# araffin/srl-zoo

Measured on AMD Instinct MI355X. Metric: images/sec (224x224x3) AE+VAE train step, higher is better.
Workload: dtype f32; 1 GPU; synthetic 224x224x3 obs, --losses autoencoder, custom_cnn, state-dim 200, bs=256 per GPU (512 frames fwd+bwd per step per GPU), Adam lr 0.005, normalised fp32 observations resident in HBM; global_batch=256, parallelism=dp1, rccl_ranks=1, devices=1

## Files before the change

srl-zoo_amd/csrc/bn_pool.hip:

```cpp
#include "common.h"

namespace {

constexpr int STAGE_ROWS = 128;

template <typename T>
__global__ __launch_bounds__(256) void reduce_rows_kernel(const T* __restrict__ rows, int nrows, double* __restrict__ out) {
  rows += (size_t)blockIdx.y * nrows * 128;
  out += (size_t)blockIdx.y * gridDim.x * 128;
  const int col = threadIdx.x & 127, half = threadIdx.x >> 7;
  double a0 = 0.0, a1 = 0.0, a2 = 0.0, a3 = 0.0;
  const int step = 2 * gridDim.x;
  int r = blockIdx.x * 2 + half;
  for (; r + 3 * step < nrows; r += 4 * step) {
    a0 += (double)rows[(size_t)r * 128 + col];
    a1 += (double)rows[(size_t)(r + step) * 128 + col];
    a2 += (double)rows[(size_t)(r + 2 * step) * 128 + col];
    a3 += (double)rows[(size_t)(r + 3 * step) * 128 + col];
  }
  for (; r < nrows; r += step) a0 += (double)rows[(size_t)r * 128 + col];
  __shared__ double sm[128];
  const double s = (a0 + a1) + (a2 + a3);
  if (half) sm[col] = s;
  __syncthreads();
  if (!half) out[(size_t)blockIdx.x * 128 + col] = s + sm[col];
}

static int stage_blocks(int nrows) {
  int g = (nrows + 7) / 8;
  if (g > STAGE_ROWS) g = STAGE_ROWS;
  return g < 1 ? 1 : g;
}

__global__ __launch_bounds__(1024) void bn_finalize_kernel(const double* __restrict__ partial, int n_partials, double count,
                                   const float* __restrict__ gamma, const float* __restrict__ beta, float eps,
                                   float momentum, int repeat, float* __restrict__ running_mean,
                                   float* __restrict__ running_var, float* __restrict__ bnp,
                                   float* __restrict__ batch_stat, int groups, long long* __restrict__ tick) {
  if (tick && blockIdx.x == 0 && threadIdx.x == 0) tick[0] += groups;
  gamma += blockIdx.x * 64; beta += blockIdx.x * 64;
  if (running_mean) running_mean += blockIdx.x * 64;
  if (running_var) running_var += blockIdx.x * 64;
  bnp += blockIdx.x * 256;
  partial += (size_t)blockIdx.x * groups * n_partials * 128;
  const int rec_stride = 256 * (int)gridDim.x;
  constexpr int NP = 16;
  const int c = threadIdx.x & 63, part = threadIdx.x >> 6;
  __shared__ double sm[2][NP][64];
  float rm = 0.f, rv = 0.f;
  const bool upd = running_mean && running_var;
  if (part == 0 && upd) { rm = running_mean[c]; rv = running_var[c]; }
  for (int g = 0; g < groups; ++g) {
    const double* pg = partial + (size_t)g * n_partials * 128;
    double s = 0.0, q = 0.0;
    for (int i = part; i < n_partials; i += NP) {
      s += pg[(size_t)i * 128 + c];
      q += pg[(size_t)i * 128 + 64 + c];
    }
    __syncthreads();
    sm[0][part][c] = s; sm[1][part][c] = q;
    __syncthreads();
    if (part == 0) {
      s = 0.0; q = 0.0;
#pragma unroll
      for (int k = 0; k < NP; ++k) { s += sm[0][k][c]; q += sm[1][k][c]; }
      const double mean = s / count;
      double var = q / count - mean * mean;
      if (var < 0.0) var = 0.0;
      const float invstd = (float)(1.0 / sqrt(var + (double)eps));
      const float ga = gamma[c], be = beta[c];
      const float scale = ga * invstd;
      float* rec = bnp + g * rec_stride;
      rec[c] = (float)mean; rec[64 + c] = invstd; rec[128 + c] = scale; rec[192 + c] = be - (float)mean * scale;
      const double unbiased = (count > 1.0) ? var * count / (count - 1.0) : var;
      if (batch_stat) { batch_stat[g * 128 + c] = (float)mean; batch_stat[g * 128 + 64 + c] = (float)unbiased; }
      for (int r = 0; r < repeat; ++r) {
        rm = (1.f - momentum) * rm + momentum * (float)mean;
        rv = (1.f - momentum) * rv + momentum * (float)unbiased;
      }
    }
  }
  if (part == 0 && upd) { running_mean[c] = rm; running_var[c] = rv; }
}

__global__ void bn_eval_params_kernel(const float* gamma, const float* beta, const float* rm, const float* rv, float eps,
                                      float* bnp) {
  const int c = threadIdx.x;
  const float invstd = 1.f / sqrtf(rv[c] + eps);
  const float scale = gamma[c] * invstd;
  bnp[c] = rm[c]; bnp[64 + c] = invstd; bnp[128 + c] = scale; bnp[192 + c] = beta[c] - rm[c] * scale;
}

__global__ void bn_replay_kernel(const float* batch_stat, float momentum, float* rm, float* rv) {
  const int c = threadIdx.x;
  rm[c] = (1.f - momentum) * rm[c] + momentum * batch_stat[c];
  rv[c] = (1.f - momentum) * rv[c] + momentum * batch_stat[64 + c];
}

__global__ __launch_bounds__(256) void bn_relu_pool_fwd_kernel(const float* __restrict__ y, const float* __restrict__ bnp,
                                                               float* __restrict__ pooled, uint8_t* __restrict__ argmax,
                                                               int N, int H, int W, int HP, int WP, int pad, int out_nchw,
                                                               int npg, int gx) {
  const int HB = (HP + 1) >> 1, WB = (WP + 1) >> 1;
  const int t = xcd_remap(blockIdx.x, gridDim.x);
  const int brow = t / gx, xb = t - brow * gx;
  const int c4 = threadIdx.x & 15;
  const int bx = (xb * blockDim.x + threadIdx.x) >> 4;
  if (bx >= WB) return;
  const int n = brow / HB, by = brow - n * HB;
  bnp += (n / npg) * 256;
  const f32x4 sc = *(const f32x4*)(bnp + 128 + c4 * 4);
  const f32x4 sh = *(const f32x4*)(bnp + 192 + c4 * 4);
  const int py0 = 2 * by, px0 = 2 * bx;
  const int iy0 = py0 * 2 - pad, ix0 = px0 * 2 - pad;
  f32x4 win[25];
  unsigned inside = 0;
#pragma unroll
  for (int r = 0; r < 5; ++r)
#pragma unroll
    for (int c = 0; c < 5; ++c) {
      const int iy = iy0 + r, ix = ix0 + c;
      const bool ok = iy >= 0 && iy < H && ix >= 0 && ix < W;
      win[r * 5 + c] = *(const f32x4*)(y + (ok ? ((size_t)(n * H + iy) * W + ix) * 64 : (size_t)0) + c4 * 4);
      inside |= (ok ? 1u : 0u) << (r * 5 + c);
    }
#pragma unroll
  for (int k = 0; k < 25; ++k) {
#pragma unroll
    for (int j = 0; j < 4; ++j) {
      float z = win[k][j] * sc[j] + sh[j];
      win[k][j] = z > 0.f ? z : 0.f;
    }
  }
#pragma unroll
  for (int dy = 0; dy < 2; ++dy)
#pragma unroll
    for (int dx = 0; dx < 2; ++dx) {
      const int py = py0 + dy, px = px0 + dx;
      if (py >= HP || px >= WP) continue;
      f32x4 best = {-1.f, -1.f, -1.f, -1.f};
      int bi[4] = {0, 0, 0, 0};
#pragma unroll
      for (int ky = 0; ky < 3; ++ky)
#pragma unroll
        for (int kx = 0; kx < 3; ++kx) {
          const int e = (2 * dy + ky) * 5 + 2 * dx + kx;
          const bool ok = (inside >> e) & 1u;
#pragma unroll
          for (int j = 0; j < 4; ++j)
            if (ok && win[e][j] > best[j]) { best[j] = win[e][j]; bi[j] = ky * 3 + kx; }
        }
      const long long pix = ((long long)n * HP + py) * WP + px;
      if (out_nchw) {
#pragma unroll
        for (int j = 0; j < 4; ++j) pooled[((size_t)(n * 64 + c4 * 4 + j) * HP + py) * WP + px] = best[j];
      } else {
        *(f32x4*)(pooled + (size_t)pix * 64 + c4 * 4) = best;
      }
      if (argmax) {
        const uint32_t packed = (uint32_t)bi[0] | ((uint32_t)bi[1] << 8) | ((uint32_t)bi[2] << 16) | ((uint32_t)bi[3] << 24);
        *(uint32_t*)(argmax + (size_t)pix * 64 + c4 * 4) = packed;
      }
    }
}

__device__ __forceinline__ void block_reduce_store(const double (&s1)[4], const double (&s2)[4], double* __restrict__ partial) {
  __shared__ double sm[16][128];
  const int c4 = threadIdx.x & 15, prow = threadIdx.x >> 4;
#pragma unroll
  for (int j = 0; j < 4; ++j) { sm[prow][c4 * 4 + j] = s1[j]; sm[prow][64 + c4 * 4 + j] = s2[j]; }
  __syncthreads();
  if (threadIdx.x < 128) {
    double s = 0.0;
#pragma unroll
    for (int r = 0; r < 16; ++r) s += sm[r][threadIdx.x];
    partial[((size_t)blockIdx.y * gridDim.x + blockIdx.x) * 128 + threadIdx.x] = s;
  }
}

__global__ __launch_bounds__(256) void bn_relu_pool_bwd_reduce(const float* __restrict__ y, const float* __restrict__ bnp,
                                                              const uint8_t* __restrict__ argmax,
                                                              const float* __restrict__ dpooled,
                                                              const float* __restrict__ pooled, double* __restrict__ partial,
                                                              int N, int H, int W, int HP, int WP, int pad, int dp_nchw) {
  bnp += blockIdx.y * 256;
  const int n0 = blockIdx.y * N;
  const int c4 = threadIdx.x & 15;
  const f32x4 mean = *(const f32x4*)(bnp + c4 * 4);
  const f32x4 invstd = *(const f32x4*)(bnp + 64 + c4 * 4);
  const f32x4 sc = *(const f32x4*)(bnp + 128 + c4 * 4);
  const f32x4 sh = *(const f32x4*)(bnp + 192 + c4 * 4);
  double s1[4] = {0.0, 0.0, 0.0, 0.0}, s2[4] = {0.0, 0.0, 0.0, 0.0};
  for (int lrow = blockIdx.x; lrow < N * HP; lrow += gridDim.x) {
    const int row = n0 * HP + lrow;
    const int n = row / HP, py = row - n * HP;
    for (int px = threadIdx.x >> 4; px < WP; px += 16) {
      const long long pix = (long long)row * WP + px;
      const uint32_t packed = *(const uint32_t*)(argmax + (size_t)pix * 64 + c4 * 4);
      f32x4 dp;
      if (dp_nchw) {
#pragma unroll
        for (int j = 0; j < 4; ++j) dp[j] = dpooled[((size_t)(n * 64 + c4 * 4 + j) * HP + py) * WP + px];
      } else {
        dp = *(const f32x4*)(dpooled + (size_t)pix * 64 + c4 * 4);
      }
      f32x4 pz = {0.f, 0.f, 0.f, 0.f};
      if (pooled) {
        if (dp_nchw) {
#pragma unroll
          for (int j = 0; j < 4; ++j) pz[j] = pooled[((size_t)(n * 64 + c4 * 4 + j) * HP + py) * WP + px];
        } else {
          pz = *(const f32x4*)(pooled + (size_t)pix * 64 + c4 * 4);
        }
      }
#pragma unroll
      for (int j = 0; j < 4; ++j) {
        float v, z;
        if (pooled && fabsf(sc[j]) > 1e-3f * fabsf(sh[j])) {
          z = pz[j];
          v = (z - sh[j]) / sc[j];
        } else {
          const int a = (packed >> (8 * j)) & 0xff;
          const int iy = py * 2 - pad + a / 3, ix = px * 2 - pad + a % 3;
          v = y[((size_t)(n * H + iy) * W + ix) * 64 + c4 * 4 + j];
          z = v * sc[j] + sh[j];
        }
        if (z > 0.f) {
          s1[j] += (double)dp[j];
          s2[j] += (double)(dp[j] * ((v - mean[j]) * invstd[j]));
        }
      }
    }
  }
  block_reduce_store(s1, s2, partial);
}

__global__ __launch_bounds__(1024) void bn_bwd_finalize(const double* __restrict__ partial, int nblocks, float* __restrict__ sums,
                                                       float* __restrict__ dgamma, float* __restrict__ dbeta, int groups) {
  const int c = threadIdx.x & 127, part = threadIdx.x >> 7;
  __shared__ double sm[8][128];
  double total = 0.0;
  for (int g = 0; g < groups; ++g) {
    const double* pg = partial + (size_t)g * nblocks * 128;
    double s = 0.0;
    for (int i = part; i < nblocks; i += 8) s += pg[(size_t)i * 128 + c];
    __syncthreads();
    sm[part][c] = s;
    __syncthreads();
    if (part == 0) {
      s = ((sm[0][c] + sm[1][c]) + (sm[2][c] + sm[3][c])) + ((sm[4][c] + sm[5][c]) + (sm[6][c] + sm[7][c]));
      sums[g * 128 + c] = (float)s;
      total = (g == 0) ? s : total + s;
    }
  }
  if (part == 0) {
    if (c < 64) { if (dbeta) dbeta[c] = (float)total; } else { if (dgamma) dgamma[c - 64] = (float)total; }
  }
}

__global__ __launch_bounds__(256) void bn_relu_pool_bwd_apply(const float* __restrict__ y, const float* __restrict__ bnp,
                                                             const uint8_t* __restrict__ argmax,
                                                             const float* __restrict__ dpooled, const float* __restrict__ sums,
                                                             float* __restrict__ dy, int N, int H, int W, int HP, int WP,
                                                             int pad, int dp_nchw, int training, float inv_count, int npg, int gx) {
  const int HB = (H + pad + 1) / 2, WB = (W + pad + 1) / 2;
  {
    const int t = xcd_remap(blockIdx.x, gridDim.x);
    const int brow = t / gx, xb = t - brow * gx;
    const int c4 = threadIdx.x & 15;
    const int bx = (xb * blockDim.x + threadIdx.x) >> 4;
    if (bx >= WB) return;
    const int n = brow / HB, by = brow - n * HB;
    bnp += (n / npg) * 256;
    sums += (n / npg) * 128;
    const f32x4 mean = *(const f32x4*)(bnp + c4 * 4);
    const f32x4 invstd = *(const f32x4*)(bnp + 64 + c4 * 4);
    const f32x4 sc = *(const f32x4*)(bnp + 128 + c4 * 4);
    const f32x4 sh = *(const f32x4*)(bnp + 192 + c4 * 4);
    f32x4 m1 = {0.f, 0.f, 0.f, 0.f}, m2 = m1;
    if (training) { m1 = *(const f32x4*)(sums + c4 * 4); m2 = *(const f32x4*)(sums + 64 + c4 * 4); }
    uint32_t am[2][2];
    f32x4 dp[2][2];
    unsigned wok = 0;
#pragma unroll
    for (int a = 0; a < 2; ++a)
#pragma unroll
      for (int b = 0; b < 2; ++b) {
        const int py = by - 1 + a, px = bx - 1 + b;
        const bool ok = py >= 0 && py < HP && px >= 0 && px < WP;
        const size_t pp = ok ? ((size_t)(n * HP + py) * WP + px) : (size_t)0;
        am[a][b] = *(const uint32_t*)(argmax + pp * 64 + c4 * 4);
        if (dp_nchw) {
#pragma unroll
          for (int j = 0; j < 4; ++j)
            dp[a][b][j] = dpooled[ok ? ((size_t)(n * 64 + c4 * 4 + j) * HP + py) * WP + px : (size_t)0];
        } else {
          dp[a][b] = *(const f32x4*)(dpooled + pp * 64 + c4 * 4);
        }
        wok |= (ok ? 1u : 0u) << (2 * a + b);
      }
    f32x4 yv[2][2];
    unsigned yok = 0;
#pragma unroll
    for (int ry = 0; ry < 2; ++ry)
#pragma unroll
      for (int rx = 0; rx < 2; ++rx) {
        const int iy = 2 * by - pad + ry, ix = 2 * bx - pad + rx;
        const bool ok = iy >= 0 && iy < H && ix >= 0 && ix < W;
        yv[ry][rx] = *(const f32x4*)(y + (ok ? ((size_t)(n * H + iy) * W + ix) * 64 : (size_t)0) + c4 * 4);
        yok |= (ok ? 1u : 0u) << (2 * ry + rx);
      }
#pragma unroll
    for (int a = 0; a < 2; ++a)
#pragma unroll
      for (int b = 0; b < 2; ++b) {
        asm volatile("" : "+v"(am[a][b]), "+v"(dp[a][b]), "+v"(yv[a][b]));
        if (!((wok >> (2 * a + b)) & 1u)) am[a][b] = 0xffffffffu;
      }
#pragma unroll
    for (int ry = 0; ry < 2; ++ry) {
      const int iy = 2 * by - pad + ry;
#pragma unroll
      for (int rx = 0; rx < 2; ++rx) {
        const int ix = 2 * bx - pad + rx;
        if (!((yok >> (2 * ry + rx)) & 1u)) continue;
        const size_t pix = ((size_t)(n * H + iy) * W + ix);
        const f32x4 v = yv[ry][rx];
        f32x4 dz = {0.f, 0.f, 0.f, 0.f};
#pragma unroll
        for (int a = (ry ? 1 : 0); a < 2; ++a) {
          const int ky = ry ? 1 : (a ? 0 : 2);
#pragma unroll
          for (int b = (rx ? 1 : 0); b < 2; ++b) {
            const int kx = rx ? 1 : (b ? 0 : 2);
            const uint32_t me = (uint32_t)(ky * 3 + kx);
#pragma unroll
            for (int j = 0; j < 4; ++j)
              if (((am[a][b] >> (8 * j)) & 0xffu) == me) dz[j] += dp[a][b][j];
          }
        }
        f32x4 o;
#pragma unroll
        for (int j = 0; j < 4; ++j) {
          const float z = v[j] * sc[j] + sh[j];
          const float d = z > 0.f ? dz[j] : 0.f;
          if (training) {
            const float xh = (v[j] - mean[j]) * invstd[j];
            o[j] = sc[j] * (d - m1[j] * inv_count - xh * m2[j] * inv_count);
          } else {
            o[j] = sc[j] * d;
          }
        }
        *(f32x4*)(dy + pix * 64 + c4 * 4) = o;
      }
    }
  }
}

__global__ __launch_bounds__(256) void bn_relu_fwd_kernel(const float* __restrict__ y, const float* __restrict__ bnp,
                                                         float* __restrict__ a, long long pixels) {
  const long long total = pixels * 16;
  for (long long id = (long long)blockIdx.x * blockDim.x + threadIdx.x; id < total; id += (long long)gridDim.x * blockDim.x) {
    const int c4 = (int)(id & 15);
    const f32x4 sc = *(const f32x4*)(bnp + 128 + c4 * 4);
    const f32x4 sh = *(const f32x4*)(bnp + 192 + c4 * 4);
    const f32x4 v = *(const f32x4*)(y + id * 4);
    f32x4 o;
#pragma unroll
    for (int j = 0; j < 4; ++j) { const float z = v[j] * sc[j] + sh[j]; o[j] = z > 0.f ? z : 0.f; }
    *(f32x4*)(a + id * 4) = o;
  }
}

__global__ __launch_bounds__(256) void bn_relu_bwd_reduce(const float* __restrict__ y, const float* __restrict__ bnp,
                                                         const float* __restrict__ da, double* __restrict__ partial,
                                                         long long pixels) {
  bnp += blockIdx.y * 256;
  y += (size_t)blockIdx.y * pixels * 64;
  da += (size_t)blockIdx.y * pixels * 64;
  const int c4 = threadIdx.x & 15;
  const f32x4 mean = *(const f32x4*)(bnp + c4 * 4);
  const f32x4 invstd = *(const f32x4*)(bnp + 64 + c4 * 4);
  const f32x4 sc = *(const f32x4*)(bnp + 128 + c4 * 4);
  const f32x4 sh = *(const f32x4*)(bnp + 192 + c4 * 4);
  double s1[4] = {0.0, 0.0, 0.0, 0.0}, s2[4] = {0.0, 0.0, 0.0, 0.0};
  for (long long pix = (long long)blockIdx.x * 16 + (threadIdx.x >> 4); pix < pixels; pix += (long long)gridDim.x * 16) {
    const f32x4 v = *(const f32x4*)(y + pix * 64 + c4 * 4);
    const f32x4 d = *(const f32x4*)(da + pix * 64 + c4 * 4);
#pragma unroll
    for (int j = 0; j < 4; ++j) {
      const float z = v[j] * sc[j] + sh[j];
      if (z > 0.f) { s1[j] += (double)d[j]; s2[j] += (double)(d[j] * ((v[j] - mean[j]) * invstd[j])); }
    }
  }
  block_reduce_store(s1, s2, partial);
}

__global__ __launch_bounds__(256) void bn_relu_bwd_apply(const float* __restrict__ y, const float* __restrict__ bnp,
                                                        const float* __restrict__ da, const float* __restrict__ sums,
                                                        float* __restrict__ dy, long long pixels, int training,
                                                        float inv_count) {
  bnp += blockIdx.y * 256;
  sums += blockIdx.y * 128;
  y += (size_t)blockIdx.y * pixels * 64;
  da += (size_t)blockIdx.y * pixels * 64;
  dy += (size_t)blockIdx.y * pixels * 64;
  const long long total = pixels * 16;
  for (long long id = (long long)blockIdx.x * blockDim.x + threadIdx.x; id < total; id += (long long)gridDim.x * blockDim.x) {
    const int c4 = (int)(id & 15);
    const f32x4 mean = *(const f32x4*)(bnp + c4 * 4);
    const f32x4 invstd = *(const f32x4*)(bnp + 64 + c4 * 4);
    const f32x4 sc = *(const f32x4*)(bnp + 128 + c4 * 4);
    const f32x4 sh = *(const f32x4*)(bnp + 192 + c4 * 4);
    const f32x4 v = *(const f32x4*)(y + id * 4);
    const f32x4 d = *(const f32x4*)(da + id * 4);
    f32x4 o;
#pragma unroll
    for (int j = 0; j < 4; ++j) {
      const float z = v[j] * sc[j] + sh[j];
      const float g = z > 0.f ? d[j] : 0.f;
      if (training) {
        const float xh = (v[j] - mean[j]) * invstd[j];
        o[j] = sc[j] * (g - sums[c4 * 4 + j] * inv_count - xh * sums[64 + c4 * 4 + j] * inv_count);
      } else {
        o[j] = sc[j] * g;
      }
    }
    *(f32x4*)(dy + id * 4) = o;
  }
}

__global__ void nchw_to_nhwc_kernel(const float* __restrict__ src, float* __restrict__ dst, int N, int C, int HW) {
  const long long total = (long long)N * C * HW;
  for (long long id = (long long)blockIdx.x * blockDim.x + threadIdx.x; id < total; id += (long long)gridDim.x * blockDim.x) {
    const int c = (int)(id % C);
    const long long t = id / C;
    const int p = (int)(t % HW);
    const long long n = t / HW;
    dst[id] = src[((size_t)n * C + c) * HW + p];
  }
}
__global__ void nhwc_to_nchw_kernel(const float* __restrict__ src, float* __restrict__ dst, int N, int C, int HW) {
  const long long total = (long long)N * C * HW;
  for (long long id = (long long)blockIdx.x * blockDim.x + threadIdx.x; id < total; id += (long long)gridDim.x * blockDim.x) {
    const int p = (int)(id % HW);
    const long long t = id / HW;
    const int c = (int)(t % C);
    const long long n = t / C;
    dst[id] = src[((size_t)n * HW + p) * C + c];
  }
}

static int grid_for(long long work_items, int per_block) {
  long long b = (work_items + per_block - 1) / per_block;
  const long long cap = 8LL * srlz_device_cus();
  if (b > cap) b = cap;
  return b < 1 ? 1 : (int)b;
}

constexpr int RED_BLOCKS = 1024;
constexpr int MAX_GROUPS = 8;
static int norm_groups(int groups) { return groups > 1 ? groups : 1; }

static int check_pool(const srlz_pool_desc* d) {
  SRLZ_REQUIRE(d != nullptr, SRLZ_ERR_NULL, "pool: null descriptor");
  SRLZ_REQUIRE(d->n > 0 && (d->pool_pad == 0 || d->pool_pad == 1), SRLZ_ERR_BAD_DESC, "pool: bad descriptor");
  SRLZ_REQUIRE(d->groups >= 0 && d->groups <= 8 && (d->groups <= 1 || d->n % d->groups == 0), SRLZ_ERR_BAD_DESC,
               "pool: n = %d is not a multiple of groups = %d", d->n, d->groups);
  SRLZ_REQUIRE(d->hp == (d->h + 2 * d->pool_pad - 3) / 2 + 1 && d->wp == (d->w + 2 * d->pool_pad - 3) / 2 + 1,
               SRLZ_ERR_BAD_DESC, "pool: pooled size %dx%d inconsistent with %dx%d pad %d", d->hp, d->wp, d->h, d->w, d->pool_pad);
  return 0;
}

}

extern "C" int srlz_bn_finalize(const float* stats_partial, int n_partials, int groups, long long count, const float* gamma,
                                const float* beta, float eps, float momentum, int repeat, float* running_mean,
                                float* running_var, long long* num_batches_tracked, float* bnp, float* batch_stat, void* ws,
                                size_t ws_bytes, srlz_stream_t stream) {
  SRLZ_REQUIRE(stats_partial && gamma && beta && bnp && ws, SRLZ_ERR_NULL, "bn_finalize: null pointer");
  const int G = norm_groups(groups);
  SRLZ_REQUIRE(n_partials > 0 && count > 0 && G <= MAX_GROUPS && n_partials % G == 0, SRLZ_ERR_BAD_DESC,
               "bn_finalize: %d partial records do not split into %d groups", n_partials, G);
  SRLZ_REQUIRE(ws_bytes >= srlz_bn_bwd_workspace(0), SRLZ_ERR_WORKSPACE, "bn_finalize: workspace too small");
  double* staged = (double*)ws;
  const int per = n_partials / G;
  const int g = stage_blocks(per);
  hipLaunchKernelGGL(reduce_rows_kernel<float>, dim3(g, G), dim3(256), 0, as_stream(stream), stats_partial, per, staged);
  SRLZ_LAUNCHED();
  hipLaunchKernelGGL(bn_finalize_kernel, dim3(1), dim3(1024), 0, as_stream(stream), (const double*)staged, g, (double)count,
                     gamma, beta, eps, momentum, repeat, running_mean, running_var, bnp, batch_stat, G, num_batches_tracked);
  SRLZ_LAUNCHED();
  return 0;
}

extern "C" size_t srlz_bn_finalize_chunks_workspace(int chunks, int groups) {
  const size_t pairs = (size_t)(chunks > 1 ? chunks : 1) * norm_groups(groups);
  const size_t need = pairs * STAGE_ROWS * 128 * sizeof(double);
  const size_t base = srlz_bn_bwd_workspace(0);
  return need > base ? need : base;
}

extern "C" int srlz_bn_finalize_chunks(const float* stats_partial, int tiles, int chunks, int groups, long long count,
                                       const float* gamma, const float* beta, float eps, float momentum, float* running_mean,
                                       float* running_var, long long* num_batches_tracked, float* bnp, void* ws, size_t ws_bytes,
                                       srlz_stream_t stream) {
  SRLZ_REQUIRE(stats_partial && gamma && beta && bnp && ws, SRLZ_ERR_NULL, "bn_finalize_chunks: null pointer");
  const int G = norm_groups(groups);
  SRLZ_REQUIRE(tiles > 0 && count > 0 && chunks >= 1 && chunks <= MAX_GROUPS && G <= MAX_GROUPS && tiles % G == 0, SRLZ_ERR_BAD_DESC,
               "bn_finalize_chunks: %d tiles, %d channel blocks, %d groups", tiles, chunks, G);
  SRLZ_REQUIRE(ws_bytes >= srlz_bn_finalize_chunks_workspace(chunks, G), SRLZ_ERR_WORKSPACE, "bn_finalize_chunks: workspace too small");
  double* staged = (double*)ws;
  const int per = tiles / G;
  const int g = stage_blocks(per);
  hipLaunchKernelGGL(reduce_rows_kernel<float>, dim3(g, chunks * G), dim3(256), 0, as_stream(stream), stats_partial, per, staged);
  SRLZ_LAUNCHED();
  hipLaunchKernelGGL(bn_finalize_kernel, dim3(chunks), dim3(1024), 0, as_stream(stream), (const double*)staged, g, (double)count,
                     gamma, beta, eps, momentum, 1, running_mean, running_var, bnp, (float*)nullptr, G, num_batches_tracked);
  SRLZ_LAUNCHED();
  return 0;
}

__global__ void bn_eval_params_chunks_kernel(const float* gamma, const float* beta, const float* rm, const float* rv, float eps,
                                             float* bnp) {
  const int c = threadIdx.x, ch = blockIdx.x * 64 + c;
  const float invstd = 1.f / sqrtf(rv[ch] + eps);
  const float scale = gamma[ch] * invstd;
  float* rec = bnp + blockIdx.x * 256;
  rec[c] = rm[ch]; rec[64 + c] = invstd; rec[128 + c] = scale; rec[192 + c] = beta[ch] - rm[ch] * scale;
}

extern "C" int srlz_bn_eval_params_chunks(const float* gamma, const float* beta, const float* running_mean,
                                          const float* running_var, float eps, int chunks, float* bnp, srlz_stream_t stream) {
  SRLZ_REQUIRE(gamma && beta && running_mean && running_var && bnp && chunks >= 1, SRLZ_ERR_NULL, "bn_eval_params_chunks: null pointer");
  hipLaunchKernelGGL(bn_eval_params_chunks_kernel, dim3(chunks), dim3(64), 0, as_stream(stream), gamma, beta, running_mean,
                     running_var, eps, bnp);
  SRLZ_LAUNCHED();
  return 0;
}

__global__ __launch_bounds__(256) void bn_add_relu_kernel(const float* __restrict__ a, const float* __restrict__ a_bnp,
                                                         const float* __restrict__ b, const float* __restrict__ b_bnp,
                                                         float* __restrict__ out, long long pixels, int chunks,
                                                         long long per_group) {
  const int q4 = chunks * 16;
  const long long total = pixels * q4;
  for (long long id = (long long)blockIdx.x * blockDim.x + threadIdx.x; id < total; id += (long long)gridDim.x * blockDim.x) {
    const int cq = (int)(id % q4);
    const int chunk = (int)(id / per_group) * chunks + (cq >> 4), c4 = cq & 15;
    const f32x4 sa = *(const f32x4*)(a_bnp + chunk * 256 + 128 + c4 * 4), ha = *(const f32x4*)(a_bnp + chunk * 256 + 192 + c4 * 4);
    const f32x4 va = *(const f32x4*)(a + id * 4);
    f32x4 vb = *(const f32x4*)(b + id * 4);
    if (b_bnp) {
      const f32x4 sb = *(const f32x4*)(b_bnp + chunk * 256 + 128 + c4 * 4), hb = *(const f32x4*)(b_bnp + chunk * 256 + 192 + c4 * 4);
#pragma unroll
      for (int j = 0; j < 4; ++j) vb[j] = vb[j] * sb[j] + hb[j];
    }
    f32x4 o;
#pragma unroll
    for (int j = 0; j < 4; ++j) { const float z = (va[j] * sa[j] + ha[j]) + vb[j]; o[j] = z > 0.f ? z : 0.f; }
    *(f32x4*)(out + id * 4) = o;
  }
}

extern "C" int srlz_bn_add_relu(const float* a, const float* a_bnp, const float* b, const float* b_bnp, float* out,
                                long long pixels, int chunks, int groups, srlz_stream_t stream) {
  SRLZ_REQUIRE(a && a_bnp && b && out, SRLZ_ERR_NULL, "bn_add_relu: null pointer");
  const int G = norm_groups(groups);
  SRLZ_REQUIRE(pixels > 0 && chunks >= 1 && pixels % G == 0, SRLZ_ERR_BAD_DESC, "bn_add_relu: %lld pixels, %d groups", pixels, G);
  hipLaunchKernelGGL(bn_add_relu_kernel, dim3(grid_for(pixels * chunks * 16, 256)), dim3(256), 0, as_stream(stream), a, a_bnp, b,
                     b_bnp, out, pixels, chunks, pixels / G * chunks * 16);
  SRLZ_LAUNCHED();
  return 0;
}

__global__ void avgpool_nhwc_kernel(const float* __restrict__ x, float* __restrict__ out, int hw, int c) {
  const int n = blockIdx.x;
  for (int ch = threadIdx.x; ch < c; ch += blockDim.x) {
    float s = 0.f;
    for (int p = 0; p < hw; ++p) s += x[((size_t)n * hw + p) * c + ch];
    out[(size_t)n * c + ch] = s / (float)hw;
  }
}

extern "C" int srlz_avgpool_nhwc(const float* x, float* out, int n, int hw, int c, srlz_stream_t stream) {
  SRLZ_REQUIRE(x && out && n > 0 && hw > 0 && c > 0, SRLZ_ERR_NULL, "avgpool: bad arguments");
  hipLaunchKernelGGL(avgpool_nhwc_kernel, dim3(n), dim3(256), 0, as_stream(stream), x, out, hw, c);
  SRLZ_LAUNCHED();
  return 0;
}

extern "C" int srlz_bn_eval_params(const float* gamma, const float* beta, const float* running_mean,
                                   const float* running_var, float eps, float* bnp, srlz_stream_t stream) {
  SRLZ_REQUIRE(gamma && beta && running_mean && running_var && bnp, SRLZ_ERR_NULL, "bn_eval_params: null pointer");
  hipLaunchKernelGGL(bn_eval_params_kernel, dim3(1), dim3(64), 0, as_stream(stream), gamma, beta, running_mean, running_var,
                     eps, bnp);
  SRLZ_LAUNCHED();
  return 0;
}

extern "C" int srlz_bn_replay(const float* batch_stat, float momentum, float* running_mean, float* running_var,
                              srlz_stream_t stream) {
  SRLZ_REQUIRE(batch_stat && running_mean && running_var, SRLZ_ERR_NULL, "bn_replay: null pointer");
  hipLaunchKernelGGL(bn_replay_kernel, dim3(1), dim3(64), 0, as_stream(stream), batch_stat, momentum, running_mean, running_var);
  SRLZ_LAUNCHED();
  return 0;
}

struct ReplayTable { srlz_bn_replay_item it[SRLZ_BN_REPLAY_MAX]; };
__global__ void bn_replay_many_kernel(const ReplayTable t, float momentum) {
  const srlz_bn_replay_item it = t.it[blockIdx.x];
  const int c = threadIdx.x;
  it.running_mean[c] = (1.f - momentum) * it.running_mean[c] + momentum * it.batch_stat[c];
  it.running_var[c] = (1.f - momentum) * it.running_var[c] + momentum * it.batch_stat[64 + c];
  if (c == 0 && it.num_batches_tracked) it.num_batches_tracked[0] += 1;
}

extern "C" int srlz_bn_replay_many(const srlz_bn_replay_item* items, int n, float momentum, srlz_stream_t stream) {
  SRLZ_REQUIRE(items && n >= 1 && n <= SRLZ_BN_REPLAY_MAX, SRLZ_ERR_BAD_DESC, "bn_replay_many: %d items (1 .. %d)", n, SRLZ_BN_REPLAY_MAX);
  ReplayTable t;
  for (int i = 0; i < n; ++i) {
    SRLZ_REQUIRE(items[i].batch_stat && items[i].running_mean && items[i].running_var, SRLZ_ERR_NULL, "bn_replay_many: null pointer");
    t.it[i] = items[i];
  }
  for (int i = n; i < SRLZ_BN_REPLAY_MAX; ++i) t.it[i] = items[0];
  hipLaunchKernelGGL(bn_replay_many_kernel, dim3(n), dim3(64), 0, as_stream(stream), t, momentum);
  SRLZ_LAUNCHED();
  return 0;
}

extern "C" int srlz_bn_relu_pool_fwd(const float* y, const float* bnp, float* pooled, uint8_t* argmax,
                                     const srlz_pool_desc* d, srlz_stream_t stream) {
  if (int rc = check_pool(d)) return rc;
  SRLZ_REQUIRE(y && bnp && pooled, SRLZ_ERR_NULL, "bn_relu_pool_fwd: null pointer");
  const int HB = (d->hp + 1) / 2, WB = (d->wp + 1) / 2;
  const int gx = (WB * 16 + 255) / 256;
  SRLZ_REQUIRE((long long)gx * d->n * HB <= 0x7fffffffLL && (long long)d->n * (d->h + 4) <= 0x7fffffffLL, SRLZ_ERR_BAD_DESC,
               "pool: %d images of %d x %d are too many for one launch", d->n, d->h, d->w);
  hipLaunchKernelGGL(bn_relu_pool_fwd_kernel, dim3(gx * d->n * HB), dim3(256), 0, as_stream(stream), y, bnp, pooled, argmax, d->n, d->h,
                     d->w, d->hp, d->wp, d->pool_pad, d->out_nchw, d->n / norm_groups(d->groups), gx);
  SRLZ_LAUNCHED();
  return 0;
}

extern "C" size_t srlz_bn_bwd_workspace(long long elems) {
  (void)elems;
  return (size_t)(RED_BLOCKS + STAGE_ROWS) * 128 * sizeof(double) + MAX_GROUPS * 128 * sizeof(float);
}

static int pool_bwd_sums(const float* y, const float* bnp, const uint8_t* argmax, const float* dpooled, const float* pooled,
                         float* sums, float* dgamma, float* dbeta, void* ws, const srlz_pool_desc* d, hipStream_t st) {
  double* partial = (double*)ws;
  double* staged = partial + RED_BLOCKS * 128;
  const int G = norm_groups(d->groups), npg = d->n / G;
  int nb = npg * d->hp;
  if (nb > RED_BLOCKS / G) nb = RED_BLOCKS / G;
  hipLaunchKernelGGL(bn_relu_pool_bwd_reduce, dim3(nb, G), dim3(256), 0, st, y, bnp, argmax, dpooled, pooled, partial, npg, d->h, d->w,
                     d->hp, d->wp, d->pool_pad, d->out_nchw);
  SRLZ_LAUNCHED();
  int sg = stage_blocks(nb);
  if (sg > STAGE_ROWS / G) sg = STAGE_ROWS / G;
  hipLaunchKernelGGL(reduce_rows_kernel<double>, dim3(sg, G), dim3(256), 0, st, (const double*)partial, nb, staged);
  SRLZ_LAUNCHED();
  hipLaunchKernelGGL(bn_bwd_finalize, dim3(1), dim3(1024), 0, st, (const double*)staged, sg, sums, dgamma, dbeta, G);
  SRLZ_LAUNCHED();
  return 0;
}

extern "C" int srlz_bn_relu_pool_bwd_sums(const float* y, const float* bnp, const uint8_t* argmax, const float* dpooled,
                                          const float* pooled, float* sums, float* dgamma, float* dbeta, void* ws,
                                          size_t ws_bytes, const srlz_pool_desc* d, srlz_stream_t stream) {
  if (int rc = check_pool(d)) return rc;
  SRLZ_REQUIRE(y && bnp && argmax && dpooled && sums && ws, SRLZ_ERR_NULL, "bn_relu_pool_bwd_sums: null pointer");
  SRLZ_REQUIRE(ws_bytes >= srlz_bn_bwd_workspace(0), SRLZ_ERR_WORKSPACE, "bn_relu_pool_bwd_sums: workspace too small");
  return pool_bwd_sums(y, bnp, argmax, dpooled, pooled, sums, dgamma, dbeta, ws, d, as_stream(stream));
}

extern "C" int srlz_bn_relu_pool_bwd(const float* y, const float* bnp, const uint8_t* argmax, const float* dpooled,
                                     const float* pooled, float* dy, float* dgamma, float* dbeta, int training, void* ws,
                                     size_t ws_bytes, const srlz_pool_desc* d, srlz_stream_t stream) {
  if (int rc = check_pool(d)) return rc;
  SRLZ_REQUIRE(y && bnp && argmax && dpooled && dy && ws, SRLZ_ERR_NULL, "bn_relu_pool_bwd: null pointer");
  SRLZ_REQUIRE(ws_bytes >= srlz_bn_bwd_workspace(0), SRLZ_ERR_WORKSPACE, "bn_relu_pool_bwd: workspace too small");
  hipStream_t st = as_stream(stream);
  float* sums = (float*)((double*)ws + (RED_BLOCKS + STAGE_ROWS) * 128);
  if (int rc = pool_bwd_sums(y, bnp, argmax, dpooled, pooled, sums, dgamma, dbeta, ws, d, st)) return rc;
  const int HB = (d->h + d->pool_pad + 1) / 2, WB = (d->w + d->pool_pad + 1) / 2;
  SRLZ_REQUIRE((long long)((WB * 16 + 255) / 256) * d->n * HB <= 0x7fffffffLL && (long long)d->n * (d->h + 2) <= 0x7fffffffLL,
               SRLZ_ERR_BAD_DESC, "pool: %d images of %d x %d are too many for one launch", d->n, d->h, d->w);
  const int npg = d->n / norm_groups(d->groups);
  const float inv_count = 1.0f / (float)((double)npg * d->h * d->w);
  const int gx = (WB * 16 + 255) / 256;
  hipLaunchKernelGGL(bn_relu_pool_bwd_apply, dim3(gx * d->n * HB), dim3(256), 0, st, y, bnp, argmax, dpooled, sums, dy,
                     d->n, d->h, d->w, d->hp, d->wp, d->pool_pad, d->out_nchw, training, inv_count, npg, gx);
  SRLZ_LAUNCHED();
  return 0;
}

extern "C" int srlz_bn_relu_pool_bwd_apply(const float* y, const float* bnp, const uint8_t* argmax, const float* dpooled,
                                           const float* sums, float* dy, int training, const srlz_pool_desc* d,
                                           srlz_stream_t stream) {
  if (int rc = check_pool(d)) return rc;
  SRLZ_REQUIRE(y && bnp && argmax && dpooled && sums && dy, SRLZ_ERR_NULL, "bn_relu_pool_bwd_apply: null pointer");
  const int HB = (d->h + d->pool_pad + 1) / 2, WB = (d->w + d->pool_pad + 1) / 2;
  SRLZ_REQUIRE((long long)((WB * 16 + 255) / 256) * d->n * HB <= 0x7fffffffLL && (long long)d->n * (d->h + 2) <= 0x7fffffffLL,
               SRLZ_ERR_BAD_DESC, "pool: %d images of %d x %d are too many for one launch", d->n, d->h, d->w);
  const int npg = d->n / norm_groups(d->groups);
  const float inv_count = 1.0f / (float)((double)npg * d->h * d->w);
  const int gx = (WB * 16 + 255) / 256;
  hipLaunchKernelGGL(bn_relu_pool_bwd_apply, dim3(gx * d->n * HB), dim3(256), 0, as_stream(stream), y, bnp, argmax,
                     dpooled, sums, dy, d->n, d->h, d->w, d->hp, d->wp, d->pool_pad, d->out_nchw, training, inv_count, npg, gx);
  SRLZ_LAUNCHED();
  return 0;
}

extern "C" int srlz_bn_relu_fwd(const float* y, const float* bnp, float* a, long long pixels, srlz_stream_t stream) {
  SRLZ_REQUIRE(y && bnp && a, SRLZ_ERR_NULL, "bn_relu_fwd: null pointer");
  hipLaunchKernelGGL(bn_relu_fwd_kernel, dim3(grid_for(pixels * 16, 256)), dim3(256), 0, as_stream(stream), y, bnp, a, pixels);
  SRLZ_LAUNCHED();
  return 0;
}

static int bn_relu_bwd_sums_launch(const float* y, const float* bnp, const float* da, float* sums, float* dgamma, float* dbeta,
                                   void* ws, long long pixels, int G, hipStream_t st) {
  SRLZ_REQUIRE(G >= 1 && G <= MAX_GROUPS && pixels % G == 0, SRLZ_ERR_BAD_DESC, "bn_relu_bwd: %lld positions do not split into %d groups",
               pixels, G);
  double* partial = (double*)ws;
  double* staged = partial + RED_BLOCKS * 128;
  const long long ppg = pixels / G;
  int nb = (int)((ppg + 15) / 16);
  if (nb > RED_BLOCKS / G) nb = RED_BLOCKS / G;
  hipLaunchKernelGGL(bn_relu_bwd_reduce, dim3(nb, G), dim3(256), 0, st, y, bnp, da, partial, ppg);
  SRLZ_LAUNCHED();
  int sg = stage_blocks(nb);
  if (sg > STAGE_ROWS / G) sg = STAGE_ROWS / G;
  hipLaunchKernelGGL(reduce_rows_kernel<double>, dim3(sg, G), dim3(256), 0, st, (const double*)partial, nb, staged);
  SRLZ_LAUNCHED();
  hipLaunchKernelGGL(bn_bwd_finalize, dim3(1), dim3(1024), 0, st, (const double*)staged, sg, sums, dgamma, dbeta, G);
  SRLZ_LAUNCHED();
  return 0;
}

extern "C" int srlz_bn_bwd_finalize_partials(const float* partial, int n_partials, int groups, float* sums, float* dgamma,
                                             float* dbeta, void* ws, size_t ws_bytes, srlz_stream_t stream) {
  SRLZ_REQUIRE(partial && sums && ws, SRLZ_ERR_NULL, "bn_bwd_finalize_partials: null pointer");
  const int G = norm_groups(groups);
  SRLZ_REQUIRE(n_partials > 0 && G <= MAX_GROUPS && n_partials % G == 0, SRLZ_ERR_BAD_DESC,
               "bn_bwd_finalize_partials: %d records do not split into %d groups", n_partials, G);
  SRLZ_REQUIRE(ws_bytes >= srlz_bn_bwd_workspace(0), SRLZ_ERR_WORKSPACE, "bn_bwd_finalize_partials: workspace too small");
  hipStream_t st = as_stream(stream);
  double* staged = (double*)ws;
  const int per = n_partials / G;
  const int g = stage_blocks(per);
  hipLaunchKernelGGL(reduce_rows_kernel<float>, dim3(g, G), dim3(256), 0, st, partial, per, staged);
  SRLZ_LAUNCHED();
  hipLaunchKernelGGL(bn_bwd_finalize, dim3(1), dim3(1024), 0, st, (const double*)staged, g, sums, dgamma, dbeta, G);
  SRLZ_LAUNCHED();
  return 0;
}

extern "C" int srlz_bn_relu_bwd_sums(const float* y, const float* bnp, const float* da, float* sums, float* dgamma,
                                     float* dbeta, void* ws, size_t ws_bytes, long long pixels, int groups,
                                     srlz_stream_t stream) {
  SRLZ_REQUIRE(y && bnp && da && sums && ws, SRLZ_ERR_NULL, "bn_relu_bwd_sums: null pointer");
  SRLZ_REQUIRE(ws_bytes >= srlz_bn_bwd_workspace(0), SRLZ_ERR_WORKSPACE, "bn_relu_bwd_sums: workspace too small");
  return bn_relu_bwd_sums_launch(y, bnp, da, sums, dgamma, dbeta, ws, pixels, norm_groups(groups), as_stream(stream));
}

extern "C" int srlz_bn_relu_bwd(const float* y, const float* bnp, const float* da, float* dy, float* dgamma, float* dbeta,
                                int training, void* ws, size_t ws_bytes, long long pixels, int groups, srlz_stream_t stream) {
  SRLZ_REQUIRE(y && bnp && da && dy && ws, SRLZ_ERR_NULL, "bn_relu_bwd: null pointer");
  SRLZ_REQUIRE(ws_bytes >= srlz_bn_bwd_workspace(0), SRLZ_ERR_WORKSPACE, "bn_relu_bwd: workspace too small");
  hipStream_t st = as_stream(stream);
  const int G = norm_groups(groups);
  float* sums = (float*)((double*)ws + (RED_BLOCKS + STAGE_ROWS) * 128);
  if (int rc = bn_relu_bwd_sums_launch(y, bnp, da, sums, dgamma, dbeta, ws, pixels, G, st)) return rc;
  const long long ppg = pixels / G;
  const float inv_count = 1.0f / (float)(double)ppg;
  hipLaunchKernelGGL(bn_relu_bwd_apply, dim3(grid_for(ppg * 16, 256), G), dim3(256), 0, st, y, bnp, da, sums, dy, ppg,
                     training, inv_count);
  SRLZ_LAUNCHED();
  return 0;
}

extern "C" int srlz_nchw_to_nhwc(const float* src, float* dst, int n, int c, int h, int w, srlz_stream_t stream) {
  SRLZ_REQUIRE(src && dst, SRLZ_ERR_NULL, "nchw_to_nhwc: null pointer");
  hipLaunchKernelGGL(nchw_to_nhwc_kernel, dim3(grid_for((long long)n * c * h * w, 256)), dim3(256), 0, as_stream(stream), src,
                     dst, n, c, h * w);
  SRLZ_LAUNCHED();
  return 0;
}

extern "C" int srlz_nhwc_to_nchw(const float* src, float* dst, int n, int c, int h, int w, srlz_stream_t stream) {
  SRLZ_REQUIRE(src && dst, SRLZ_ERR_NULL, "nhwc_to_nchw: null pointer");
  hipLaunchKernelGGL(nhwc_to_nchw_kernel, dim3(grid_for((long long)n * c * h * w, 256)), dim3(256), 0, as_stream(stream), src,
                     dst, n, c, h * w);
  SRLZ_LAUNCHED();
  return 0;
}
```

Before: 44950 images/s.

## Fuse BN partial-row staging reduction and finalize into one kernel

Replaces the two-kernel sequence (staged reduce_rows then a single-block finalize) with one fused kernel per BN reduction. Each block handles a few channels and reproduces the same two-level staged sum order in shared memory before computing the batch-norm record. The forward stats path and the partial-finalize path fall back to the old kernels above a row threshold. This removes a launch and a global round trip per BN layer in forward and backward. The cost is fewer, larger blocks, with each one re-reading the partial rows for only a handful of columns.

```diff
diff --git a/srl-zoo_amd/csrc/bn_pool.hip b/srl-zoo_amd/csrc/bn_pool.hip
--- a/srl-zoo_amd/csrc/bn_pool.hip
+++ b/srl-zoo_amd/csrc/bn_pool.hip
@@ -30,6 +30,23 @@
   int g = (nrows + 7) / 8;
   if (g > STAGE_ROWS) g = STAGE_ROWS;
   return g < 1 ? 1 : g;
+}
+
+__device__ __forceinline__ void bn_channel_record(double s, double q, double count, float ga, float be, float eps, float momentum,
+                                                  int repeat, float* __restrict__ rec, float* __restrict__ stat, int c, float& rm,
+                                                  float& rv) {
+  const double mean = s / count;
+  double var = q / count - mean * mean;
+  if (var < 0.0) var = 0.0;
+  const float invstd = (float)(1.0 / sqrt(var + (double)eps));
+  const float scale = ga * invstd;
+  rec[c] = (float)mean; rec[64 + c] = invstd; rec[128 + c] = scale; rec[192 + c] = be - (float)mean * scale;
+  const double unbiased = (count > 1.0) ? var * count / (count - 1.0) : var;
+  if (stat) { stat[c] = (float)mean; stat[64 + c] = (float)unbiased; }
+  for (int r = 0; r < repeat; ++r) {
+    rm = (1.f - momentum) * rm + momentum * (float)mean;
+    rv = (1.f - momentum) * rv + momentum * (float)unbiased;
+  }
 }
 
 __global__ __launch_bounds__(1024) void bn_finalize_kernel(const double* __restrict__ partial, int n_partials, double count,
@@ -64,23 +81,76 @@
       s = 0.0; q = 0.0;
 #pragma unroll
       for (int k = 0; k < NP; ++k) { s += sm[0][k][c]; q += sm[1][k][c]; }
-      const double mean = s / count;
-      double var = q / count - mean * mean;
-      if (var < 0.0) var = 0.0;
-      const float invstd = (float)(1.0 / sqrt(var + (double)eps));
-      const float ga = gamma[c], be = beta[c];
-      const float scale = ga * invstd;
-      float* rec = bnp + g * rec_stride;
-      rec[c] = (float)mean; rec[64 + c] = invstd; rec[128 + c] = scale; rec[192 + c] = be - (float)mean * scale;
-      const double unbiased = (count > 1.0) ? var * count / (count - 1.0) : var;
-      if (batch_stat) { batch_stat[g * 128 + c] = (float)mean; batch_stat[g * 128 + 64 + c] = (float)unbiased; }
-      for (int r = 0; r < repeat; ++r) {
-        rm = (1.f - momentum) * rm + momentum * (float)mean;
-        rv = (1.f - momentum) * rv + momentum * (float)unbiased;
-      }
+      bn_channel_record(s, q, count, gamma[c], beta[c], eps, momentum, repeat, bnp + g * rec_stride, batch_stat ? batch_stat + g * 128 : nullptr,
+                        c, rm, rv);
     }
   }
   if (part == 0 && upd) { running_mean[c] = rm; running_var[c] = rv; }
+}
+
+constexpr int FZ_NC = 4;
+constexpr int FZ_SLOTS = 1024 / FZ_NC;
+static_assert(FZ_SLOTS >= 2 * STAGE_ROWS, "one pass covers every block and half of the first stage");
+
+template <typename T>
+__device__ __forceinline__ void fz_stage(const T* __restrict__ rows, int nrows, int g, int col, double (*stA)[FZ_NC],
+                                         double (*stB)[FZ_NC]) {
+  const int j = threadIdx.x % FZ_NC, v = threadIdx.x / FZ_NC;
+  if (v < 2 * g) {
+    double a0 = 0.0, a1 = 0.0, a2 = 0.0, a3 = 0.0;
+    const int step = 2 * g;
+    int r = v;
+    for (; r + 3 * step < nrows; r += 4 * step) {
+      a0 += (double)rows[(size_t)r * 128 + col];
+      a1 += (double)rows[(size_t)(r + step) * 128 + col];
+      a2 += (double)rows[(size_t)(r + 2 * step) * 128 + col];
+      a3 += (double)rows[(size_t)(r + 3 * step) * 128 + col];
+    }
+    for (; r < nrows; r += step) a0 += (double)rows[(size_t)r * 128 + col];
+    stA[v][j] = (a0 + a1) + (a2 + a3);
+  }
+  __syncthreads();
+  if (v < g) stB[v][j] = stA[2 * v][j] + stA[2 * v + 1][j];
+  __syncthreads();
+}
+
+__global__ __launch_bounds__(1024) void bn_finalize_fused_kernel(const float* __restrict__ rows, int nrows, int g, double count,
+                                   const float* __restrict__ gamma, const float* __restrict__ beta, float eps,
+                                   float momentum, int repeat, float* __restrict__ running_mean,
+                                   float* __restrict__ running_var, float* __restrict__ bnp,
+                                   float* __restrict__ batch_stat, int groups, long long* __restrict__ tick) {
+  if (tick && blockIdx.x == 0 && blockIdx.y == 0 && threadIdx.x == 0) tick[0] += groups;
+  gamma += blockIdx.y * 64; beta += blockIdx.y * 64;
+  if (running_mean) running_mean += blockIdx.y * 64;
+  if (running_var) running_var += blockIdx.y * 64;
+  bnp += blockIdx.y * 256;
+  rows += (size_t)blockIdx.y * groups * nrows * 128;
+  const int rec_stride = 256 * (int)gridDim.y;
+  constexpr int CB = FZ_NC / 2, NP = 16;
+  __shared__ double stA[FZ_SLOTS][FZ_NC], stB[STAGE_ROWS][FZ_NC], sp[NP][FZ_NC];
+  const int t = threadIdx.x, j = t % FZ_NC;
+  const int col = (j < CB) ? blockIdx.x * CB + j : 64 + blockIdx.x * CB + (j - CB);
+  const int c = blockIdx.x * CB + t;
+  float rm = 0.f, rv = 0.f;
+  const bool upd = running_mean && running_var;
+  if (t < CB && upd) { rm = running_mean[c]; rv = running_var[c]; }
+  for (int grp = 0; grp < groups; ++grp) {
+    fz_stage(rows + (size_t)grp * nrows * 128, nrows, g, col, stA, stB);
+    if (t < NP * FZ_NC) {
+      double s = 0.0;
+      for (int i = t / FZ_NC; i < g; i += NP) s += stB[i][j];
+      sp[t / FZ_NC][j] = s;
+    }
+    __syncthreads();
+    if (t < CB) {
+      double s = 0.0, q = 0.0;
+#pragma unroll
+      for (int k = 0; k < NP; ++k) { s += sp[k][t]; q += sp[k][CB + t]; }
+      bn_channel_record(s, q, count, gamma[c], beta[c], eps, momentum, repeat, bnp + grp * rec_stride,
+                        batch_stat ? batch_stat + grp * 128 : nullptr, c, rm, rv);
+    }
+  }
+  if (t < CB && upd) { running_mean[c] = rm; running_var[c] = rv; }
 }
 
 __global__ void bn_eval_params_kernel(const float* gamma, const float* beta, const float* rm, const float* rv, float eps,
@@ -255,6 +325,32 @@
   }
   if (part == 0) {
     if (c < 64) { if (dbeta) dbeta[c] = (float)total; } else { if (dgamma) dgamma[c - 64] = (float)total; }
+  }
+}
+
+template <typename T>
+__global__ __launch_bounds__(1024) void bn_bwd_finalize_fused(const T* __restrict__ rows, int nrows, int g, float* __restrict__ sums,
+                                                             float* __restrict__ dgamma, float* __restrict__ dbeta, int groups) {
+  __shared__ double stA[FZ_SLOTS][FZ_NC], stB[STAGE_ROWS][FZ_NC], sp[8][FZ_NC];
+  const int t = threadIdx.x, j = t % FZ_NC;
+  const int col = blockIdx.x * FZ_NC + j;
+  double total = 0.0;
+  for (int grp = 0; grp < groups; ++grp) {
+    fz_stage(rows + (size_t)grp * nrows * 128, nrows, g, col, stA, stB);
+    if (t < 8 * FZ_NC) {
+      double s = 0.0;
+      for (int i = t / FZ_NC; i < g; i += 8) s += stB[i][j];
+      sp[t / FZ_NC][j] = s;
+    }
+    __syncthreads();
+    if (t < FZ_NC) {
+      const double s = ((sp[0][t] + sp[1][t]) + (sp[2][t] + sp[3][t])) + ((sp[4][t] + sp[5][t]) + (sp[6][t] + sp[7][t]));
+      sums[grp * 128 + col] = (float)s;
+      total = (grp == 0) ? s : total + s;
+    }
+  }
+  if (t < FZ_NC) {
+    if (col < 64) { if (dbeta) dbeta[col] = (float)total; } else { if (dgamma) dgamma[col - 64] = (float)total; }
   }
 }
 
@@ -462,6 +558,11 @@
 constexpr int MAX_GROUPS = 8;
 static int norm_groups(int groups) { return groups > 1 ? groups : 1; }
 
+#ifndef SRLZ_BN_FUSED_MAX_ROWS
+#define SRLZ_BN_FUSED_MAX_ROWS 2048
+#endif
+constexpr long long FUSED_MAX_ROWS = SRLZ_BN_FUSED_MAX_ROWS;
+
 static int check_pool(const srlz_pool_desc* d) {
   SRLZ_REQUIRE(d != nullptr, SRLZ_ERR_NULL, "pool: null descriptor");
   SRLZ_REQUIRE(d->n > 0 && (d->pool_pad == 0 || d->pool_pad == 1), SRLZ_ERR_BAD_DESC, "pool: bad descriptor");
@@ -486,6 +587,13 @@
   double* staged = (double*)ws;
   const int per = n_partials / G;
   const int g = stage_blocks(per);
+  if (n_partials <= FUSED_MAX_ROWS) {
+    hipLaunchKernelGGL(bn_finalize_fused_kernel, dim3(64 / (FZ_NC / 2)), dim3(1024), 0, as_stream(stream), stats_partial, per, g,
+                       (double)count, gamma, beta, eps, momentum, repeat, running_mean, running_var, bnp, batch_stat, G,
+                       num_batches_tracked);
+    SRLZ_LAUNCHED();
+    return 0;
+  }
   hipLaunchKernelGGL(reduce_rows_kernel<float>, dim3(g, G), dim3(256), 0, as_stream(stream), stats_partial, per, staged);
   SRLZ_LAUNCHED();
   hipLaunchKernelGGL(bn_finalize_kernel, dim3(1), dim3(1024), 0, as_stream(stream), (const double*)staged, g, (double)count,
@@ -513,6 +621,13 @@
   double* staged = (double*)ws;
   const int per = tiles / G;
   const int g = stage_blocks(per);
+  if (tiles <= FUSED_MAX_ROWS) {
+    hipLaunchKernelGGL(bn_finalize_fused_kernel, dim3(64 / (FZ_NC / 2), chunks), dim3(1024), 0, as_stream(stream), stats_partial, per, g,
+                       (double)count, gamma, beta, eps, momentum, 1, running_mean, running_var, bnp, (float*)nullptr, G,
+                       num_batches_tracked);
+    SRLZ_LAUNCHED();
+    return 0;
+  }
   hipLaunchKernelGGL(reduce_rows_kernel<float>, dim3(g, chunks * G), dim3(256), 0, as_stream(stream), stats_partial, per, staged);
   SRLZ_LAUNCHED();
   hipLaunchKernelGGL(bn_finalize_kernel, dim3(chunks), dim3(1024), 0, as_stream(stream), (const double*)staged, g, (double)count,
@@ -651,7 +766,6 @@
 static int pool_bwd_sums(const float* y, const float* bnp, const uint8_t* argmax, const float* dpooled, const float* pooled,
                          float* sums, float* dgamma, float* dbeta, void* ws, const srlz_pool_desc* d, hipStream_t st) {
   double* partial = (double*)ws;
-  double* staged = partial + RED_BLOCKS * 128;
   const int G = norm_groups(d->groups), npg = d->n / G;
   int nb = npg * d->hp;
   if (nb > RED_BLOCKS / G) nb = RED_BLOCKS / G;
@@ -660,9 +774,8 @@
   SRLZ_LAUNCHED();
   int sg = stage_blocks(nb);
   if (sg > STAGE_ROWS / G) sg = STAGE_ROWS / G;
-  hipLaunchKernelGGL(reduce_rows_kernel<double>, dim3(sg, G), dim3(256), 0, st, (const double*)partial, nb, staged);
-  SRLZ_LAUNCHED();
-  hipLaunchKernelGGL(bn_bwd_finalize, dim3(1), dim3(1024), 0, st, (const double*)staged, sg, sums, dgamma, dbeta, G);
+  hipLaunchKernelGGL(bn_bwd_finalize_fused<double>, dim3(128 / FZ_NC), dim3(1024), 0, st, (const double*)partial, nb, sg, sums, dgamma,
+                     dbeta, G);
   SRLZ_LAUNCHED();
   return 0;
 }
@@ -726,7 +839,6 @@
   SRLZ_REQUIRE(G >= 1 && G <= MAX_GROUPS && pixels % G == 0, SRLZ_ERR_BAD_DESC, "bn_relu_bwd: %lld positions do not split into %d groups",
                pixels, G);
   double* partial = (double*)ws;
-  double* staged = partial + RED_BLOCKS * 128;
   const long long ppg = pixels / G;
   int nb = (int)((ppg + 15) / 16);
   if (nb > RED_BLOCKS / G) nb = RED_BLOCKS / G;
@@ -734,9 +846,8 @@
   SRLZ_LAUNCHED();
   int sg = stage_blocks(nb);
   if (sg > STAGE_ROWS / G) sg = STAGE_ROWS / G;
-  hipLaunchKernelGGL(reduce_rows_kernel<double>, dim3(sg, G), dim3(256), 0, st, (const double*)partial, nb, staged);
-  SRLZ_LAUNCHED();
-  hipLaunchKernelGGL(bn_bwd_finalize, dim3(1), dim3(1024), 0, st, (const double*)staged, sg, sums, dgamma, dbeta, G);
+  hipLaunchKernelGGL(bn_bwd_finalize_fused<double>, dim3(128 / FZ_NC), dim3(1024), 0, st, (const double*)partial, nb, sg, sums, dgamma,
+                     dbeta, G);
   SRLZ_LAUNCHED();
   return 0;
 }
@@ -752,6 +863,11 @@
   double* staged = (double*)ws;
   const int per = n_partials / G;
   const int g = stage_blocks(per);
+  if (n_partials <= FUSED_MAX_ROWS) {
+    hipLaunchKernelGGL(bn_bwd_finalize_fused<float>, dim3(128 / FZ_NC), dim3(1024), 0, st, partial, per, g, sums, dgamma, dbeta, G);
+    SRLZ_LAUNCHED();
+    return 0;
+  }
   hipLaunchKernelGGL(reduce_rows_kernel<float>, dim3(g, G), dim3(256), 0, st, partial, per, staged);
   SRLZ_LAUNCHED();
   hipLaunchKernelGGL(bn_bwd_finalize, dim3(1), dim3(1024), 0, st, (const double*)staged, g, sums, dgamma, dbeta, G);
```

Measured after the change: 44990 images/s (median of 4 runs). Within noise of the previous version (+0.1%).
